# MarSaKi/VLN-BEVBert

Hardware: AMD Instinct MI355X
Metric: pretrain_samples_per_sec (higher is better)
Workload: dtype bf16+fp32-residual

## Files before the change

### include/bevbert_hip.h

```cpp
#ifndef BEVBERT_HIP_H
#define BEVBERT_HIP_H

#include <stdint.h>

#ifdef __cplusplus
extern "C" {
#endif

typedef struct ihipStream_t* hipStream_t;

#define BEVBERT_F32 0
#define BEVBERT_BF16 1
#define BEVBERT_F16 2

const char* bevbert_last_error(void);
int bevbert_version(void);
int bevbert_hip_error_reset(void);
const char* bevbert_arch(void);
const char* bevbert_attn_last_path(int backward);

int bevbert_bev_lift_bin(const float* depths, const float* T_c2w, const float* T_w2c, const float* S_w2c,
                         const float* pix_scale, int B, int V, int hw, float depth_scale, int dim, float res,
                         float y_clip, int* cell, int* order, int* cell_start, hipStream_t stream);
int bevbert_bev_bin_points(const float* points, const uint8_t* drop_mask, int B, int P, int dim, float res,
                           float y_clip, int* cell, int* order, int* cell_start, hipStream_t stream);
int bevbert_bev_splat_mean(const void* feat, int feat_dtype, const int* order, const int* cell_start, void* out,
                           int out_dtype, int B, int P, int K, int C, const uint8_t* sem_ids, const double* sem_dense,
                           int S, uint8_t* out_sem, uint8_t* out_sem_mask, const int* sample_rows, int rows_per_sample,
                           hipStream_t stream);

int bevbert_attn_fwd(const void* q, const void* k, const void* v, void* o, float* lse, const float* key_mask,
                     const float* bias, const int64_t* strides, int B, int nh, int Lq, int Lk, int head_dim,
                     float scale, int dtype, int impl, float drop_p, uint64_t seed, uint64_t offset,
                     uint64_t* drop_bits, int bits_ready, hipStream_t stream);
int bevbert_attn_bwd(const void* q, const void* k, const void* v, const void* o, const void* dout, const float* lse,
                     float* delta_ws, void* dq, void* dk, void* dv, float* dbias, const float* key_mask,
                     const float* bias, const int64_t* strides, int B, int nh, int Lq, int Lk, int head_dim,
                     float scale, int dtype, int impl, float drop_p, uint64_t seed, uint64_t offset,
                     const uint64_t* drop_bits, hipStream_t stream);
int64_t bevbert_attn_drop_bits_words(int B, int nh, int Lq, int Lk);
int bevbert_attn_drop_bits(uint64_t* drop_bits, int B, int nh, int Lq, int Lk, float drop_p, uint64_t seed,
                           uint64_t offset, hipStream_t stream);

int bevbert_bias_dropout_residual_layernorm_fwd(const void* x, const float* bias, const void* residual,
                                                const float* gamma, const float* beta, void* y, void* z_out,
                                                float* mean, float* rstd, int rows, int H, float eps, int dtype,
                                                float drop_p, uint64_t seed, uint64_t offset, hipStream_t stream);
int bevbert_layernorm_post_fwd(const void* x, const float* bias, const float* gamma, const float* beta,
                               const void* post1, const void* post2, void* y, void* z_out, float* mean, float* rstd,
                               int rows, int H, float eps, int dtype, hipStream_t stream);
int bevbert_layernorm_bwd(const void* dy, const void* z, const float* mean, const float* rstd, const float* gamma,
                          void* dz, void* dx, float* dgamma, float* dbeta, float* dbias, float* workspace, int rows,
                          int H, int dtype, float drop_p, uint64_t seed, uint64_t offset, int accumulate,
                          hipStream_t stream);
int bevbert_layernorm_bwd_add(const void* dy, const void* z, const float* mean, const float* rstd, const float* gamma,
                              void* dz, void* dx, const void* dz_add, float* dgamma, float* dbeta, float* dbias,
                              float* workspace, int rows, int H, int dtype, float drop_p, uint64_t seed, uint64_t offset,
                              int accumulate, hipStream_t stream);
int bevbert_layernorm_res32_fwd(const void* x, const float* bias, const void* residual, int residual_dtype,
                                const float* gamma, const float* beta, void* y16, float* y32, float* z32, float* mean,
                                float* rstd, int rows, int H, float eps, float drop_p, uint64_t seed, uint64_t offset,
                                hipStream_t stream);
// ... 180 lines not shown
```

### vln_bevbert_amd/csrc/attn_common.h

```cpp
#pragma once
#include "common.h"

#define ATTN_D 64

struct AttnArgs {
  const void *q, *k, *v;
  void* o;
  float* lse;
  const float* key_mask;
  const float* bias;
  int64_t ldq, ldk, ldv, ldo;
  int64_t bsq, bsk, bsv, bso;
  int B, nh, Lq, Lk;
  float scale;
  float drop_p;
  float keep_scale;
  uint32_t drop_thr;
  uint32_t drop_key;
  const uint32_t* salt;
  int nblk;
  int Lk2;
  uint64_t* drop_bits;
  uint64_t* drop_bits_b;
  int nq16, nk64;
  const void* dout;
  const float* delta;
  void *dq, *dk, *dv;
  float* dbias;
  int dbg;
};

__device__ __forceinline__ void attn_decode_block(const AttnArgs& a, int& blk, int& h, int& b) {
  const int nwg = gridDim.x, id = blockIdx.x;
  const int q = nwg >> 3, r = nwg & 7, xcd = id & 7, slot = id >> 3;
  const int w = (xcd < r ? xcd * (q + 1) : r * (q + 1) + (xcd - r) * q) + slot;
  blk = w % a.nblk;
  const int t = w / a.nblk;
  h = t % a.nh;
  b = t / a.nh;
}

__device__ __forceinline__ size_t attn_bits_word(const AttnArgs& a, int bh, int q16, int k64, int t, int r) {
  return ((((size_t)bh * a.nq16 + q16) * a.nk64 + k64) * 4 + t) * 4 + r;
}

__device__ __forceinline__ uint32_t attn_row_base(const AttnArgs& a, int b, int h, int q) {
  return (uint32_t)((((uint32_t)b * a.nh + h) * a.Lq + q) * (uint32_t)a.Lk2);
}
__device__ __forceinline__ uint32_t attn_elem(const AttnArgs& a, int b, int h, int q, int k) {
  return attn_row_base(a, b, h, q) + (uint32_t)k;
}
```

### vln_bevbert_amd/csrc/attn_short.hip

```cpp
#include "attn_mfma_common.h"

typedef const __attribute__((address_space(4))) uint64_t* sh_cu64p;

template <int CTRL> __device__ __forceinline__ float sh_dpp(float v) {
  return __int_as_float(__builtin_amdgcn_update_dpp(0, __float_as_int(v), CTRL, 0xf, 0xf, true));
}
__device__ __forceinline__ float sh_sum8(float v) {
  v += sh_dpp<0xB1>(v);
  v += sh_dpp<0x4E>(v);
  return v + sh_dpp<0x141>(v);
}
__device__ __forceinline__ bf16x8 sh_join(uint2 a, uint2 b) { return as_bf16x8(make_uint4(a.x, a.y, b.x, b.y)); }
__device__ __forceinline__ uint2 sh_pack4(const f32x4& v) {
  return make_uint2(pack_bf16x2(v[0], v[1]), pack_bf16x2(v[2], v[3]));
}
template <bool HI>
__device__ __forceinline__ bf16x8 sh_frag_tr(const bf16_raw* img, int stride, int row_lo, int row_hi, int col0, int lane) {
  const int i = lane & 15;
  const int off = (i >> 2) * stride + col0 + 4 * (i & 3);
  const uint2 lo = lds_tr16(img + row_lo * stride + off);
  uint2 hi = make_uint2(0u, 0u);
  if (HI) hi = lds_tr16(img + row_hi * stride + off);
  return as_bf16x8(make_uint4(lo.x, lo.y, hi.x, hi.y));
}

#define SH_ST_LD 72
__device__ __forceinline__ void sh_store_tile(bf16_raw* stage, const f32x4 (&acc)[4], float mul, bf16_raw* gtile, int64_t ld,
                                              int nrows, int lane) {
  const int g = lane >> 4, c = lane & 15;
#pragma unroll
  for (int dt = 0; dt < 4; ++dt)
    *reinterpret_cast<uint2*>(stage + c * SH_ST_LD + dt * 16 + g * 4) =
        make_uint2(pack_bf16x2(acc[dt][0] * mul, acc[dt][1] * mul), pack_bf16x2(acc[dt][2] * mul, acc[dt][3] * mul));
#pragma unroll
  for (int i = 0; i < 2; ++i) {
    const int row = (lane >> 3) + 8 * i, ch = lane & 7;
    const uint4 v = *reinterpret_cast<const uint4*>(stage + row * SH_ST_LD + ch * 8);
    if (row < nrows) *reinterpret_cast<uint4*>(gtile + (size_t)row * ld + ch * 8) = v;
  }
}

template <int NKT, int DROP>
__global__ __launch_bounds__(512) void attn_short_fwd_kernel(AttnArgs a) {
  constexpr int NC = (NKT + 1) / 2;
  __shared__ __attribute__((aligned(16))) bf16_raw s_k[16 * NKT * LDT];
  __shared__ __attribute__((aligned(16))) bf16_raw s_v[16 * NKT * LDT];
  __shared__ __attribute__((aligned(16))) float s_mk[16 * NKT];
  extern __shared__ __attribute__((aligned(16))) bf16_raw s_stage[];
  const int tid = threadIdx.x, lane = tid & 63, g = lane >> 4, c = lane & 15;
  const int w = __builtin_amdgcn_readfirstlane(tid >> 6), nw = blockDim.x >> 6;
  int blk, h, b;
  attn_decode_block(a, blk, h, b);
  const int bh = b * a.nh + h;
  if (DROP == 1) a.drop_key = bb_salted(a.drop_key, a.salt);
  const bf16_raw* qp = (const bf16_raw*)a.q + (size_t)b * a.bsq + h * ATTN_D;
  const bf16_raw* kp = (const bf16_raw*)a.k + (size_t)b * a.bsk + h * ATTN_D;
  const bf16_raw* vp = (const bf16_raw*)a.v + (size_t)b * a.bsv + h * ATTN_D;
  const float sc2 = a.scale * LOG2E, inv_sc2 = 1.0f / sc2;

  const int qt = blk * nw + w;
  const int qrow = qt * 16 + c;
  const int qr = qrow < a.Lq ? qrow : a.Lq - 1;
  bf16x8 qf[2];
// ... 182 lines not shown
      if (row < 16 * NQT) {
        *reinterpret_cast<uint4*>(s_q + row * LDT + ch * 8) = qv[i];
        *reinterpret_cast<uint4*>(s_do + row * LDT + ch * 8) = dv[i];
        const uint32_t dw[4] = {dv[i].x, dv[i].y, dv[i].z, dv[i].w}, ow[4] = {ov[i].x, ov[i].y, ov[i].z, ov[i].w};
        float dsum = 0.f;
#pragma unroll
        for (int j = 0; j < 4; ++j)
          dsum += __uint_as_float(dw[j] << 16) * __uint_as_float(ow[j] << 16) +
                  __uint_as_float(dw[j] & 0xffff0000u) * __uint_as_float(ow[j] & 0xffff0000u);
        dsum = sh_sum8(dsum);
        if ((lane & 7) == 0) s_dlt[row] = dsum;
      }
    }
  }
  if (tid < 16 * NQT) s_lse2[tid] = tid < a.Lq ? a.lse[(size_t)bh * a.Lq + tid] * LOG2E : INFINITY;
  if (tid < 16 * NKT) {
    float m = -INFINITY;
    if (tid < a.Lk) m = a.key_mask ? a.key_mask[(size_t)b * a.Lk + tid] * LOG2E : 0.f;
    s_mk[tid] = m;
  }
  __syncthreads();

  const f32x4 zero = (f32x4){0.f, 0.f, 0.f, 0.f};
  f32x4 dk[4], dv[4];
  if (w < NKT) {
    const bf16x8 kb0 = lds_frag_rows(s_k, t, 0, lane), kb1 = lds_frag_rows(s_k, t, 1, lane);
    const float mk2 = s_mk[t * 16 + c];
  #pragma unroll
    for (int dt = 0; dt < 4; ++dt) dk[dt] = dv[dt] = zero;
#pragma unroll
    for (int m = 0; m < NCQ; ++m) {
      uint2 pp[2] = {make_uint2(0u, 0u), make_uint2(0u, 0u)}, pds[2] = {make_uint2(0u, 0u), make_uint2(0u, 0u)};
#pragma unroll
      for (int j = 0; j < 2; ++j) {
        const int qt = 2 * m + j;
        if (qt < NQT) {
          f32x4 s = mfma16(lds_frag_rows(s_q, qt, 0, lane), kb0, zero);
          s = mfma16(lds_frag_rows(s_q, qt, 1, lane), kb1, s);
          f32x4 dp = mfma16(lds_frag_rows(s_do, qt, 0, lane), vb[0], zero);
          dp = mfma16(lds_frag_rows(s_do, qt, 1, lane), vb[1], dp);
          const float4 l4 = *reinterpret_cast<const float4*>(s_lse2 + 16 * qt + 4 * g);
          const float4 d4 = *reinterpret_cast<const float4*>(s_dlt + 16 * qt + 4 * g);
          const float lrow[4] = {l4.x, l4.y, l4.z, l4.w}, drow[4] = {d4.x, d4.y, d4.z, d4.w};
          uint32_t kbits = 0xfu;
          if (DROP) kbits = (uint32_t)(bw[qt < NQT ? qt : 0] >> (16 * (c >> 2) + 4 * g));
          f32x4 pd, dsv;
// ... 28 lines not shown
  }
  __syncthreads();
  constexpr bool STAGED = NR * 16 * SH_ST_LD * 2 <= 2 * 16 * NQT * LDT * 2;
  bf16_raw* const stage = s_q + w * 16 * SH_ST_LD;
  if (w < NKT) {
    const int key = t * 16 + c;
    if (STAGED) {
      if (t * 16 < a.Lk && !(a.dbg & 1)) {
        bf16_raw* dkp = (bf16_raw*)a.dk + (size_t)b * a.bsk + (size_t)(t * 16) * a.ldk + h * ATTN_D;
        bf16_raw* dvp = (bf16_raw*)a.dv + (size_t)b * a.bsv + (size_t)(t * 16) * a.ldv + h * ATTN_D;
        sh_store_tile(stage, dk, a.scale, dkp, a.ldk, a.Lk - t * 16, lane);
        sh_store_tile(stage, dv, 1.0f, dvp, a.ldv, a.Lk - t * 16, lane);
      }
    } else if (key < a.Lk && !((a.dbg & 1) && lane != 0)) {
      bf16_raw* dkp = (bf16_raw*)a.dk + (size_t)b * a.bsk + (size_t)key * a.ldk + h * ATTN_D;
      bf16_raw* dvp = (bf16_raw*)a.dv + (size_t)b * a.bsv + (size_t)key * a.ldv + h * ATTN_D;
#pragma unroll
      for (int dt = 0; dt < 4; ++dt) {
        st4<bf16_raw>(dkp + dt * 16 + g * 4, make_float4(dk[dt][0] * a.scale, dk[dt][1] * a.scale, dk[dt][2] * a.scale,
                                                          dk[dt][3] * a.scale));
        st4<bf16_raw>(dvp + dt * 16 + g * 4, make_float4(dv[dt][0], dv[dt][1], dv[dt][2], dv[dt][3]));
      }
    }
  }
  if (w < NQT && w * 16 < a.Lq) {
    const int qt = w;
    f32x4 dq[4];
#pragma unroll
    for (int dt = 0; dt < 4; ++dt) dq[dt] = zero;
#pragma unroll
    for (int m = 0; m < NCK; ++m) {
      if (2 * m + 1 < NKT) {
        const bf16x8 dsf = sh_frag_tr<true>(s_ds, DS_LD, 32 * m + 4 * g, 32 * m + 16 + 4 * g, 16 * qt, lane);
#pragma unroll
        for (int dt = 0; dt < 4; ++dt)
          dq[dt] = mfma16(sh_frag_tr<true>(s_k, LDT, 32 * m + 4 * g, 32 * m + 16 + 4 * g, dt * 16, lane), dsf, dq[dt]);
      } else {
        const bf16x8 dsf = sh_frag_tr<false>(s_ds, DS_LD, 32 * m + 4 * g, 0, 16 * qt, lane);
#pragma unroll
        for (int dt = 0; dt < 4; ++dt)
          dq[dt] = mfma16(sh_frag_tr<false>(s_k, LDT, 32 * m + 4 * g, 0, dt * 16, lane), dsf, dq[dt]);
      }
    }
    const int qrow = qt * 16 + c;
    if (STAGED) {
      if (!(a.dbg & 1)) {
        bf16_raw* dqp = (bf16_raw*)a.dq + (size_t)b * a.bsq + (size_t)(qt * 16) * a.ldq + h * ATTN_D;
        sh_store_tile(stage, dq, a.scale, dqp, a.ldq, a.Lq - qt * 16, lane);
      }
    } else if (qrow < a.Lq && !((a.dbg & 1) && lane != 0)) {
      bf16_raw* dqp = (bf16_raw*)a.dq + (size_t)b * a.bsq + (size_t)qrow * a.ldq + h * ATTN_D;
#pragma unroll
      for (int dt = 0; dt < 4; ++dt)
        st4<bf16_raw>(dqp + dt * 16 + g * 4, make_float4(dq[dt][0] * a.scale, dq[dt][1] * a.scale,
                                                          dq[dt][2] * a.scale, dq[dt][3] * a.scale));
    }
  }
}

#define SH_MAX_LEN 96

static bool sh_aligned(const AttnArgs& a) {
  return a.ldq % 8 == 0 && a.ldk % 8 == 0 && a.ldv % 8 == 0 && a.ldo % 8 == 0 && a.bsq % 8 == 0 && a.bsk % 8 == 0 &&
         a.bsv % 8 == 0 && a.bso % 8 == 0 && ((uintptr_t)a.q % 16) == 0 && ((uintptr_t)a.k % 16) == 0 &&
         ((uintptr_t)a.v % 16) == 0 && ((uintptr_t)a.o % 16) == 0;
}

static int sh_round_tiles(int n) {
  return n <= 2 ? 2 : n <= 3 ? 3 : n <= 5 ? 5 : 6;
}

static bool sh_on() {
  const char* v = getenv("BEVBERT_ATTN_SHORT");
  return !(v && v[0] == '0');
}

bool attn_short_fwd_supported(const AttnArgs& a, bool bits_ready) {
  if (!sh_on()) return false;
// ... 72 lines not shown
```

### vln_bevbert_amd/csrc/capi.hip

```cpp
#include <stdarg.h>

#include "attn_common.h"

static thread_local char g_err[512] = "";

void bb_set_error(const char* fmt, ...) {
  va_list ap;
  va_start(ap, fmt);
  vsnprintf(g_err, sizeof(g_err), fmt, ap);
  va_end(ap);
}

BEVBERT_API const char* bevbert_last_error(void) { return g_err; }
BEVBERT_API int bevbert_hip_error_reset(void) {
  int n = 0;
  while (hipGetLastError() != hipSuccess && n < 16) ++n;
  return n;
}

BEVBERT_API int bevbert_zero(void* p, int64_t bytes, hipStream_t stream) {
  BB_REQUIRE(p != nullptr && bytes >= 0, "zero: null pointer or negative size");
  if (bytes == 0) return BB_OK;
  hipError_t e = hipMemsetAsync(p, 0, (size_t)bytes, stream);
  if (e != hipSuccess) {
    bb_set_error("zero: hipMemsetAsync failed: %s", hipGetErrorString(e));
    return BB_ELAUNCH;
  }
  return BB_OK;
}

BEVBERT_API int bevbert_version(void) { return 112; }

static const uint32_t* g_step_salt = nullptr;
const uint32_t* bb_step_salt() { return g_step_salt; }
BEVBERT_API int bevbert_set_step_salt(const void* device_word) {
  g_step_salt = static_cast<const uint32_t*>(device_word);
  return BB_OK;
}
BEVBERT_API const char* bevbert_arch(void) { return "gfx950"; }

int attn_simple_fwd(const AttnArgs& a, int dtype, hipStream_t st);
int attn_simple_bwd(const AttnArgs& a, int dtype, hipStream_t st);
int attn_delta(const AttnArgs& a, float* delta, int dtype, hipStream_t st);
int attn_mfma_fwd(const AttnArgs& a, hipStream_t st);
int attn_mfma_bwd(const AttnArgs& a, hipStream_t st);
int attn_mfma_bwd1(const AttnArgs& a, hipStream_t st);
bool attn_mfma_bwd1_supported(const AttnArgs& a);
int attn_fwd2(const AttnArgs& a, hipStream_t st);
bool attn_fwd2_supported(const AttnArgs& a);
int attn_drop_bits(const AttnArgs& a, uint64_t* bits_f, uint64_t* bits_b, uint32_t* bits_l, hipStream_t st);
int attn_fwd4(const AttnArgs& a, const uint32_t* bits_l, hipStream_t st);
bool attn_fwd4_supported(const AttnArgs& a, const uint32_t* bits_l);
int attn_bwd2(const AttnArgs& a, hipStream_t st);
bool attn_bwd2_supported(const AttnArgs& a);
// ... 69 lines not shown
  const int im = pick_impl(dtype, impl);
  if (im == 2 || im == 3) {
    BB_REQUIRE(dtype == BB_BF16, "attn_fwd: the MFMA path takes bf16 tensors");
    static const bool gen1 = [] { const char* v = getenv("BEVBERT_ATTN_FWD"); return v && v[0] == '1'; }();
    if (!gen1 && !small_kernels_on() && attn_short_fwd_supported(a, bits_ready != 0))
      return ATTN_PATH(0, "attn_short_fwd", attn_short_fwd(a, bits_ready != 0, stream));
    if (!gen1 && small_kernels_on() && attn_small_fwd_supported(a)) return ATTN_PATH(0, "attn_small_fwd", attn_small_fwd(a, stream));
    const bool small = drop_p > 0.f && (int64_t)Lq * Lk < 32768 && Lk <= 256 && !bits_ready;
    if (!gen1 && !small && attn_fwd2_supported(a)) {
      uint32_t* bits_l = drop_bits ? reinterpret_cast<uint32_t*>(drop_bits + 2 * bits_words_one(B, nh, Lq, Lk)) : nullptr;
      if (drop_p > 0.f && !bits_ready) {
        rc = attn_drop_bits(a, a.drop_bits, a.drop_bits_b, bits_l, stream);
        if (rc != BB_OK) return rc;
      }
      if (attn_fwd4_supported(a, bits_l)) return ATTN_PATH(0, "attn_fwd4", attn_fwd4(a, bits_l, stream));
      return ATTN_PATH(0, "attn_fwd2", attn_fwd2(a, stream));
    }
    return ATTN_PATH(0, "attn_mfma_fwd", attn_mfma_fwd(a, stream));
  }
  if (attn_f32_supported(a, dtype, false)) return ATTN_PATH(0, "attn_f32_fwd", attn_f32_fwd(a, stream));
  return ATTN_PATH(0, "attn_simple_fwd", attn_simple_fwd(a, dtype, stream));
}

BEVBERT_API int bevbert_attn_bwd(const void* q, const void* k, const void* v, const void* o, const void* dout,
                                 const float* lse, float* delta_ws, void* dq, void* dk, void* dv, float* dbias,
                                 const float* key_mask, const float* bias, const int64_t* strides, int B, int nh,
                                 int Lq, int Lk, int head_dim, float scale, int dtype, int impl, float drop_p,
                                 uint64_t seed, uint64_t offset, const uint64_t* drop_bits, hipStream_t stream) {
  AttnArgs a;
  int rc = fill_common(a, q, k, v, key_mask, bias, strides, B, nh, Lq, Lk, head_dim, scale, drop_p, seed, offset);
  if (rc != BB_OK) return rc;
  a.drop_bits = const_cast<uint64_t*>(drop_bits);
  a.drop_bits_b = drop_bits ? a.drop_bits + bits_words_one(B, nh, Lq, Lk) : nullptr;
  BB_REQUIRE(dtype == BB_F32 || dtype == BB_BF16, "attn_bwd: dtype %d unsupported", dtype);
  BB_REQUIRE(lse != nullptr && delta_ws != nullptr, "attn_bwd: lse and the (B,nh,Lq) delta workspace are required");
  a.o = const_cast<void*>(o); a.dout = dout; a.lse = const_cast<float*>(lse); a.delta = delta_ws;
  a.dq = dq; a.dk = dk; a.dv = dv; a.dbias = dbias;
  const int im = pick_impl(dtype, impl);
  if (im == 2 || im == 3) {
    BB_REQUIRE(dtype == BB_BF16, "attn_bwd: the MFMA path takes bf16 tensors");
    static const bool split = [] { const char* v = getenv("BEVBERT_ATTN_BWD"); return v && v[0] == 's'; }();
    static const bool gen1 = [] { const char* v = getenv("BEVBERT_ATTN_BWD"); return v && v[0] == '1'; }();
    if (!split && !gen1 && im == 2 && !small_kernels_on() && attn_short_bwd_supported(a))
      return ATTN_PATH(1, "attn_short_bwd", attn_short_bwd(a, stream));
    if (!split && !gen1 && im == 2 && small_bwd2_on() && attn_small_bwd2_supported(a)) return ATTN_PATH(1, "attn_small_bwd2", attn_small_bwd2(a, stream));
    if (!split && !gen1 && small_kernels_on() && im == 2 && attn_small_bwd_supported(a)) return ATTN_PATH(1, "attn_small_bwd", attn_small_bwd(a, stream));
    static const bool gen3 = [] { const char* v = getenv("BEVBERT_ATTN_BWD3"); return !(v && v[0] == '0'); }();
    if (!split && !gen1 && gen3 && im == 2 && attn_bwd3_supported(a)) return ATTN_PATH(1, "attn_bwd3", attn_bwd3(a, stream));
    if (!split && !gen1 && im == 2 && attn_bwd2_supported(a)) return ATTN_PATH(1, "attn_bwd2", attn_bwd2(a, stream));
    if (!split && im == 2 && attn_mfma_bwd1_supported(a)) return ATTN_PATH(1, "attn_mfma_bwd1", attn_mfma_bwd1(a, stream));
    return ATTN_PATH(1, "attn_mfma_bwd", attn_mfma_bwd(a, stream));
  }
  rc = attn_delta(a, delta_ws, dtype, stream);
  if (rc != BB_OK) return rc;
  if (attn_f32_supported(a, dtype, true)) return ATTN_PATH(1, "attn_f32_bwd", attn_f32_bwd(a, stream));
  return ATTN_PATH(1, "attn_simple_bwd", attn_simple_bwd(a, dtype, stream));
}

__global__ void keep_mask_kernel(uint8_t* out, size_t n, uint32_t key, uint32_t thr, const uint32_t* salt) {
  key = bb_salted(key, salt);
  for (size_t i = (size_t)blockIdx.x * 256 + threadIdx.x; i < n; i += (size_t)gridDim.x * 256)
    out[i] = (uint8_t)bb_keep(key, (uint32_t)i, thr);
}
BEVBERT_API int64_t bevbert_attn_drop_bits_words(int B, int nh, int Lq, int Lk) {
  return 3 * bits_words_one(B, nh, Lq, Lk);
}

// ... 22 lines not shown
```

### vln_bevbert_amd/lib.py

```python
import ctypes
import os
import re
import subprocess

import torch

_HERE = os.path.dirname(os.path.abspath(__file__))
LIB_PATH = os.path.join(_HERE, "libbevbert_hip.so")
CSRC = os.path.join(_HERE, "csrc")
EXTRA_FLAGS = {"attn_fwd4.hip": ["-fno-slp-vectorize"]}
SOURCES = ["splat.hip", "rowops.hip", "attn_simple.hip", "attn_f32.hip", "attn_mfma.hip", "attn_bwd1.hip", "attn_fwd2.hip", "attn_fwd4.hip", "attn_bwd2.hip", "attn_bwd3.hip", "attn_small.hip", "attn_short.hip", "smallk.hip", "sap_loss.hip", "graph_nav.hip", "nav_expert.hip", "gemm.hip", "capi.hip"]
HEADER = os.path.join(os.path.dirname(_HERE), "include", "bevbert_hip.h")

F32, BF16, F16 = 0, 1, 2
_DT = {torch.float32: F32, torch.bfloat16: BF16, torch.float16: F16}


class BevBertHipError(RuntimeError):
    pass


def dtype_code(t):
    try:
        return _DT[t.dtype if torch.is_tensor(t) else t]
# ... 23 lines not shown
            print(" ".join(cmd), flush=True)
        subprocess.run(cmd, check=True, cwd=CSRC)

    with ThreadPoolExecutor(max_workers=min(8, max(1, len(jobs)))) as ex:
        list(ex.map(run, jobs))
    run([hipcc, "--offload-arch=gfx950", "-shared", "-fPIC", "-o", LIB_PATH] + objs + ["-lhipblaslt"])
    return LIB_PATH


def header_symbols():
    with open(HEADER) as f:
        return sorted(set(re.findall(r"\b(bevbert_\w+)\s*\(", f.read())))


_lib = None
_P, _I, _I64, _U64, _F = ctypes.c_void_p, ctypes.c_int, ctypes.c_int64, ctypes.c_uint64, ctypes.c_float

_PROTOS = {
    "bevbert_bev_lift_bin": [_P, _P, _P, _P, _P, _I, _I, _I, _F, _I, _F, _F, _P, _P, _P, _P],
    "bevbert_bev_bin_points": [_P, _P, _I, _I, _I, _F, _F, _P, _P, _P, _P],
    "bevbert_bev_splat_mean": [_P, _I, _P, _P, _P, _I, _I, _I, _I, _I, _P, _P, _I, _P, _P, _P, _I, _P],
    "bevbert_attn_fwd": [_P, _P, _P, _P, _P, _P, _P, _P, _I, _I, _I, _I, _I, _F, _I, _I, _F, _U64, _U64, _P, _I, _P],
    "bevbert_attn_drop_bits": [_P, _I, _I, _I, _I, _F, _U64, _U64, _P],
    "bevbert_attn_bwd": [_P, _P, _P, _P, _P, _P, _P, _P, _P, _P, _P, _P, _P, _P, _I, _I, _I, _I, _I, _F, _I, _I, _F,
                         _U64, _U64, _P, _P],
    "bevbert_bias_dropout_residual_layernorm_fwd": [_P, _P, _P, _P, _P, _P, _P, _P, _P, _I, _I, _F, _I, _F, _U64,
                                                    _U64, _P],
    "bevbert_layernorm_post_fwd": [_P, _P, _P, _P, _P, _P, _P, _P, _P, _P, _I, _I, _F, _I, _P],
    "bevbert_layernorm_bwd": [_P, _P, _P, _P, _P, _P, _P, _P, _P, _P, _P, _I, _I, _I, _F, _U64, _U64, _I, _P],
    "bevbert_layernorm_res32_fwd": [_P, _P, _P, _I, _P, _P, _P, _P, _P, _P, _P, _I, _I, _F, _F, _U64, _U64, _P],
    "bevbert_layernorm_res32_bwd": [_P, _P, _P, _P, _P, _P, _P, _P, _P, _P, _P, _P, _I, _I, _F, _U64, _U64, _I, _I, _P],
    "bevbert_colsum_any": [_P, _P, _I, _I, _I, _I, _P],
    "bevbert_sem_select": [_P, _P, _I, _I, _I, _P, _P, _P, _P],
    "bevbert_bce_rows_fwd": [_P, _P, _P, _P, _I, _I, _I, _P],
    "bevbert_bce_rows_bwd": [_P, _P, _P, _P, _P, _I, _I, _I, _P],
    "bevbert_weighted_mean_fwd": [_P, _P, _P, _F, _I, _P, _P],
    "bevbert_weighted_mean_bwd": [_P, _P, _P, _F, _I, _P, _P],
    "bevbert_layernorm_bwd_add": [_P, _P, _P, _P, _P, _P, _P, _P, _P, _P, _P, _P, _I, _I, _I, _F, _U64, _U64, _I, _P],
    "bevbert_embed_sum_layernorm_fwd": [_P, _P, _P, _P, _P, _P, _P, _P, _P, _P, _I, _I, _I, _F, _I, _F, _U64, _U64, _P],
    "bevbert_embedding_grad": [_P, _P, _P, _I, _I, _I, _I, _P],
    "bevbert_rows_gather": [_P, _P, _P, _I, _I, _I, _P],
    "bevbert_graph_bias_fwd": [_P, _P, _P, _P, _I64, _P],
    "bevbert_graph_bias_bwd": [_P, _P, _I, _I, _I, _I, _P, _P, _P, _P],
    "bevbert_smallk_linear_layernorm_fwd": [_P] * 11 + [_I, _I, _I, _F, _I, _P],
    "bevbert_smallk_linear_layernorm_bwd": [_P] * 12 + [_I, _I, _I, _I, _P],
    "bevbert_rows_scatter": [_P, _P, _P, _I, _I, _I, _I, _P],
# ... 122 lines not shown
```

### vln_bevbert_amd/ops_attention.py

```python
import math
import os as _os

import torch

from .lib import dtype_code, ptr, stream
from .ops_core import ATTN_BITS, HEAD_DIM, RT, _drop_bits_words, _mark_touched, _sink, call


def _strides(q, k, v, o):
    for t in (q, k, v, o):
        assert t.dim() == 3 and t.stride(2) == 1, "attention operands are (B, L, nh*64) with unit inner stride"
    import ctypes
    arr = (ctypes.c_int64 * 8)(q.stride(1), k.stride(1), v.stride(1), o.stride(1),
                               q.stride(0), k.stride(0), v.stride(0), o.stride(0))
    return arr


class _Attention(torch.autograd.Function):

    @staticmethod
    def forward(ctx, mode, a, b_, c_, key_mask, bias, nh, drop_p, impl):
        if mode == "self":
            H = a.shape[-1] // 3
            q, k, v = a[..., :H], a[..., H:2 * H], a[..., 2 * H:]
        elif mode == "cross":
            H = a.shape[-1]
            q, k, v = a, b_[..., :H], b_[..., H:]
        else:
            H = a.shape[-1]
# ... 37 lines not shown
            dq, dk, dv = da[..., :H], da[..., H:2 * H], da[..., 2 * H:]
            grads = (da, None, None)
        elif mode == "cross":
            H = a.shape[-1]
            q, k, v = a, b_[..., :H], b_[..., H:]
            dq = torch.empty_like(a)
            dkv = ctx.kv_slot[0].grad_slice(ctx.kv_slot[1], b_) if ctx.kv_slot is not None else torch.empty_like(b_)
            dk, dv = dkv[..., :H], dkv[..., H:]
            grads = (dq, dkv, None)
        else:
            q, k, v = a, b_, c_
            dq, dk, dv = torch.empty_like(a), torch.empty_like(b_), torch.empty_like(c_)
            grads = (dq, dk, dv)
        B, Lq, Lk = q.shape[0], q.shape[1], k.shape[1]
        delta = torch.empty(B, nh, Lq, dtype=torch.float32, device=q.device)
        slot = ctx.bias_slot
        if bias is not None and ctx.needs_input_grad[5] and slot is not None and Lq == Lk:
            dbias_h = slot[0].slot(slot[1], B, Lq, q.device)
        else:
            slot = None
            dbias_h = torch.zeros(B, nh, Lq, Lk, dtype=torch.float32, device=q.device) \
                if (bias is not None and ctx.needs_input_grad[5]) else None
        assert do.shape == o.shape
        call("bevbert_attn_bwd", ptr(q), ptr(k), ptr(v), ptr(o), ptr(do), ptr(lse), ptr(delta), ptr(dq), ptr(dk),
             ptr(dv), ptr(dbias_h), ptr(key_mask), ptr(bias), _strides(q, k, v, o), B, nh, Lq, Lk, HEAD_DIM, scale,
             dtype_code(q), impl, drop_p, seed, off, ptr(bits), stream())
        if slot is not None:
            dbias = slot[0].dummy
        else:
            dbias = None if dbias_h is None else dbias_h.sum(1)
        return (None,) + grads + (None, dbias, None, None, None)


class _BiasGradHolder:

    def __init__(self, layers, nh):
        self.layers, self.nh, self.buf, self.dummy = layers, nh, None, None

    def slot(self, i, B, G, device):
        if self.buf is None:
            self.buf = torch.empty(self.layers, B, self.nh, G, G, dtype=torch.float32, device=device)
            call("bevbert_zero", ptr(self.buf), self.buf.numel() * 4, stream())
            self.dummy = torch.zeros((), dtype=torch.float32, device=device).expand(B, G, G)
        return self.buf[i]


class _GraphBias(torch.autograd.Function):

    @staticmethod
    def forward(ctx, dists, weight, bias, layers, nh):
        dists = dists.to(torch.float32).contiguous()
        out = torch.empty_like(dists)
        call("bevbert_graph_bias_fwd", ptr(dists), ptr(weight), ptr(bias), ptr(out), dists.numel(), stream())
        ctx.save_for_backward(dists)
# ... 64 lines not shown
```

### vln_bevbert_amd/ops_gemm.py

```python
import os as _os

import torch
import torch.nn.functional as F

from . import lib
from .lib import dtype_code, ptr, stream
from .ops_core import RT, _LT_WS_BYTES, _compute, _gemm, _mark_touched, _sink, call
from .ops_reduce import ReduceQueue, WgradStream, _on_launch_stream, _partial_rows


_LT_ENABLED = _os.environ.get("BEVBERT_LT_GEMM", "1") == "1"


_LT_AUTOTUNE = int(_os.environ.get("BEVBERT_LT_AUTOTUNE", "32"))


_LT_UNSUPPORTED = set()


_LT_PLAN_BUDGET = int(_os.environ.get("BEVBERT_LT_PLAN_BUDGET", "8192"))


_LT_PLANS = {}


GEMM_FALLBACKS = {}


def _warn_fallback(kind, M, N, K, why="no direct hipBLASLt plan"):
    key = (kind, int(M), int(N), int(K))
    n = GEMM_FALLBACKS.get(key, 0)
# ... 156 lines not shown
    M, N = dy2.shape
    K = x2.shape[1]
    if dy2.dtype == torch.float32 and not (_LT_ENABLED and dy2.is_cuda):
        if dy2.is_cuda:
            _warn_fallback("wgrad", N, K, M, "BEVBERT_LT_GEMM=0")
        _gemm("wgrad", lambda: _on_launch_stream(lambda: sink.addmm_(dy2.t(), x2)), N, K, M)
        return None
    S = _split_k(M, N, K) if dy2.dtype != torch.float32 else 1
    if not (S > 1 and dy2.is_contiguous() and x2.is_contiguous()):
        S = 1
    batched = WgradStream.DEFER_FINALIZE and (N * K) % 4 == 0 and dy2.is_cuda
    part = _gemm("wgrad", lambda: _linear_wgrad(dy2, x2, S, scratch=batched), N, K, M)
    if batched:
        ReduceQueue.add_accum(part.data_ptr(), sink.data_ptr(), S, N * K, dtype_code(part))
        WgradStream._keep.append(part)
        return None
    if (N * K) % 4 == 0:
        call("bevbert_accum_partials", ptr(part), ptr(sink), S, N * K, dtype_code(part), stream())
    else:
        _on_launch_stream(lambda: sink.add_(part if S == 1 else part.sum(0)))
    return part


def _param_grads(w_sink, b_sink, dyc, xc):
    if w_sink is not None:
        part = _wgrad_into(w_sink, dyc, xc)
        if part is not None and lib._override is not None:
            WgradStream._keep.append(part)
    if b_sink is not None:
        C = dyc.shape[1]
        if WgradStream.DEFER_FINALIZE and dyc.shape[0] > 0:
            nb = _partial_rows(dyc.shape[0])
            part = RT.scratch.alloc(nb * C * 4, dyc.device)
            call("bevbert_colsum_partials", ptr(dyc), part, dyc.shape[0], C, dtype_code(dyc), stream())
            ReduceQueue.add(part, nb, 1, C, (ptr(b_sink), None, None))
        else:
            ws = RT.workspace(dyc.device, lib.load().bevbert_colsum_workspace_floats(C))
            call("bevbert_colsum", ptr(dyc), ptr(b_sink), ptr(ws), dyc.shape[0], C, dtype_code(dyc), 1, stream())


class _Linear(torch.autograd.Function):

    @staticmethod
    def forward(ctx, x, weight, bias, w_c, b_c, tap=False):
        y = _gemm("fwd", lambda: _linear_fwd(x, w_c, b_c), x.numel() // x.shape[-1], w_c.shape[0], w_c.shape[1])
        ctx.save_for_backward(x, w_c)
        ctx.params = (weight, bias)
        ctx.tap = tap
        ctx.set_materialize_grads(False)
        return (y, x.view_as(x)) if tap else y

    @staticmethod
# ... 16 lines not shown
            if C % 4 != 0:
                dyc = dy2 if dy2.is_contiguous() else dy2.contiguous()
                if b_sink is not None and dyc.is_cuda:
                    _mark_touched(bias)
                    call("bevbert_colsum_any", ptr(dyc), ptr(b_sink), dyc.shape[0], C, dtype_code(dyc), 1, stream())
                    b_sink = None
                elif b_sink is not None:
                    _mark_touched(bias)
                    b_sink.add_(dy2.float().sum(0))
                    b_sink = None
                else:
                    gb = dy2.float().sum(0).to(bias.dtype)
            else:
                ws = RT.workspace(dy.device, lib.load().bevbert_colsum_workspace_floats(C))
                dyc = dy2 if dy2.is_contiguous() else dy2.contiguous()
                t = torch.empty(C, dtype=torch.float32, device=dy.device)
                call("bevbert_colsum", ptr(dyc), ptr(t), ptr(ws), dyc.shape[0], C, dtype_code(dyc), 0, stream())
                gb = t.to(bias.dtype)
        if w_sink is not None or b_sink is not None:
            dyc = dy2 if dy2.is_contiguous() else dy2.contiguous()
            xc = x2 if x2.is_contiguous() else x2.contiguous()
            if w_sink is not None:
                _mark_touched(weight)
            if b_sink is not None:
                _mark_touched(bias)
            WgradStream.submit(dy.device, lambda: _param_grads(w_sink, b_sink, dyc, xc), dyc, xc, dy)
        return dx, gw, gb, None, None, None


def linear(x, weight, bias=None, w_c=None, b_c=None):
    if w_c is None:
        w_c = _compute(weight)
    if bias is not None and b_c is None:
        b_c = _compute(bias)
    return _Linear.apply(x, weight, bias, w_c, b_c)


def linear_res(x, weight, bias=None):
    if not (x.requires_grad and torch.is_grad_enabled()) or getattr(x, "_res32", None) is not None:
        return linear(x, weight, bias), x
    return _Linear.apply(x, weight, bias, _compute(weight), None if bias is None else _compute(bias), True)


class _PackedParam:

    def __init__(self, params, compute, main_grad):
        self.params, self.compute, self.main_grad = params, compute, main_grad
        self.requires_grad = any(p.requires_grad for p in params)
        self.dtype = params[0].dtype
# ... 10 lines not shown
        ctx.save_for_backward(x)
        ctx.packed = (pw, pb)
        y = _gemm("fwd", lambda: _linear_fwd(x, pw.compute, pb.compute), x.numel() // x.shape[-1],
                  pw.compute.shape[0], pw.compute.shape[1])
        ctx.set_materialize_grads(False)
        return (y, x.view_as(x)) if tap else y

    @staticmethod
    def backward(ctx, dy, dres=None):
        (x,) = ctx.saved_tensors
        pw, pb = ctx.packed
        if dy is None:
            return dres, None, None, None
        dy2 = dy.reshape(-1, dy.shape[-1])
        x2 = x.reshape(-1, x.shape[-1])
        M, N, K = dy2.shape[0], dy2.shape[1], x2.shape[1]
        dx = _gemm("dgrad", lambda: _linear_dgrad(dy2, pw.compute, dres), M, K, N).view(x.shape) if ctx.needs_input_grad[0] else None
        if pw.requires_grad:
            pw.touch()
            pb.touch()
            C = dy2.shape[1]
            dyc = dy2 if dy2.is_contiguous() else dy2.contiguous()
            xc = x2 if x2.is_contiguous() else x2.contiguous()
            WgradStream.submit(dy.device, lambda: _param_grads(pw.main_grad, pb.main_grad, dyc, xc), dyc, xc, dy)
        return dx, None, None, None


def linear_packed(x, pw, pb):
    return _LinearPacked.apply(x, pw, pb)


HOIST_KV = _os.environ.get("BEVBERT_HOIST_KV", "1") == "1"


class _KVGradHolder:

    def __init__(self, n_layers, width):
        self.n, self.width, self.buf = n_layers, width, None

    def grad_slice(self, layer, like):
        if self.buf is None:
            self.buf = torch.empty(like.shape[:-1] + (self.n * self.width,), dtype=like.dtype, device=like.device)
        return self.buf[..., layer * self.width:(layer + 1) * self.width]


class _HoistedKV(torch.autograd.Function):

    @staticmethod
    def forward(ctx, x, pw, pb, n_layers):
        ctx.save_for_backward(x)
        ctx.packed = (pw, pb)
        y = _gemm("fwd", lambda: _linear_fwd(x, pw.compute, pb.compute), x.numel() // x.shape[-1],
                  pw.compute.shape[0], pw.compute.shape[1])
        width = y.shape[-1] // n_layers
        ctx.holder = _KVGradHolder(n_layers, width)
        return tuple(y[..., i * width:(i + 1) * width] for i in range(n_layers))

    @staticmethod
    def backward(ctx, *grads):
        (x,) = ctx.saved_tensors
        pw, pb = ctx.packed
        h = ctx.holder
        some = next((g for g in grads if g is not None), None)
        if some is None:
            return None, None, None, None
        for i, g in enumerate(grads):
            dst = h.grad_slice(i, some)
            if g is None:
                dst.zero_()
            elif g.data_ptr() != dst.data_ptr() or g.stride() != dst.stride():
                dst.copy_(g)
        dy2 = h.buf.reshape(-1, h.buf.shape[-1])
        x2 = x.reshape(-1, x.shape[-1])
        M, N, K = dy2.shape[0], dy2.shape[1], x2.shape[1]
        dx = _gemm("dgrad", lambda: _linear_dgrad(dy2, pw.compute), M, K, N).view(x.shape) if ctx.needs_input_grad[0] else None
        if pw.requires_grad:
            pw.touch()
            pb.touch()
            xc = x2 if x2.is_contiguous() else x2.contiguous()
            WgradStream.submit(dy2.device, lambda: _param_grads(pw.main_grad, pb.main_grad, dy2, xc), dy2, xc, h.buf)
        return dx, None, None, None


def hoisted_kv(context, pw, pb, n_layers):
    outs = _HoistedKV.apply(context, pw, pb, n_layers)
    if torch.is_grad_enabled() and any(o.requires_grad for o in outs):
        holder = outs[0].grad_fn.holder if hasattr(outs[0].grad_fn, "holder") else None
        if holder is not None:
            for i, o in enumerate(outs):
                o._kv_grad_slot = (holder, i)
    return outs


def linear_packed_res(x, pw, pb):
    if not (x.requires_grad and torch.is_grad_enabled()) or getattr(x, "_res32", None) is not None:
        return _LinearPacked.apply(x, pw, pb), x
    return _LinearPacked.apply(x, pw, pb, True)


def gemm_plan_count():
    return int(lib.load().bevbert_gemm_plan_count())
```

### vln_bevbert_amd/ops_reduce.py

```python
import math
import os as _os

import torch

from . import lib
from .lib import stream
from .ops_core import ATTN_BITS, Branches, RT, call


def join_captured_side_streams(extra=()):
    if not torch.cuda.is_available() or not torch.cuda.is_current_stream_capturing():
        return 0
    cur = torch.cuda.current_stream()
    seen, n = {cur.cuda_stream}, 0
    cands = [ATTN_BITS.stream] + list(Branches._streams.values()) + list(WgradStream.streams) + list(extra)
    for st in cands:
        if st is None or st.cuda_stream in seen:
            continue
        seen.add(st.cuda_stream)
        with torch.cuda.stream(st):
            capturing = torch.cuda.is_current_stream_capturing()
        if capturing:
            cur.wait_stream(st)
            n += 1
# ... 80 lines not shown
    def flush_all(cls):
        if ReduceQueue.jobs or ReduceQueue.accum_jobs:
            dev = torch.device("cuda", torch.cuda.current_device())
            if cls.active(dev):
                h = lib.stream()
                slot = cls._pending.get(h)
                if slot is None:
                    slot = cls._pending[h] = (torch.cuda.current_stream(dev), [])
                slot[1].append(lambda: ReduceQueue.flush(dev))
                mine = slot
                for other in cls._pending.values():
                    if other is not mine:
                        cls._flush(other)
                cls._flush(mine, final=True)
                return
            ReduceQueue.wait_producers(torch.cuda.current_stream(dev))
            ReduceQueue.flush(dev)
        for slot in cls._pending.values():
            cls._flush(slot)

    @classmethod
    def release(cls):
        cls._keep.clear()

    @classmethod
    def drop_pending(cls):
        for _, fns in cls._pending.values():
            fns.clear()
        cls._keep.clear()


class ScratchRing:

    INITIAL = 256 << 20

    def __init__(self, nbytes=1 << 30, max_total=64 << 30):
        self.nbytes = nbytes
        self.max_total = max(max_total, nbytes)
        self.size = 0
        self.buf = None
        self.base = 0
        self.off = 0
        self.ci = 0
        self._chunks = []
        self._old = []

    def reset(self):
        self.off = self.ci = 0
        if self._chunks:
            self.buf, self.base, self.size = self._chunks[0]

    def total_bytes(self):
# ... 214 lines not shown
```

Baseline: 3628.

## Fuse bias-gradient column sums of dQ/dK/dV into short attention backward kernel

The short attention backward kernel now also computes per-batch column sums of dQ, dK and dV, rounded to bf16, through DPP reductions and an LDS pass. These are written as partial rows into scratch buffers. The Python side arms these buffers before the call and registers them under the gradient tensor's identity. Downstream linear backward paths then feed the precomputed partials to the bias reduction instead of re-reading the full dy. This removes a separate pass over the gradient activations for the QKV bias grads, at the cost of extra kernel work, a barrier, thread-local C state and key matching on data pointers.

```diff
diff --git a/include/bevbert_hip.h b/include/bevbert_hip.h
--- a/include/bevbert_hip.h
+++ b/include/bevbert_hip.h
@@ -38,6 +38,8 @@
                      const float* bias, const int64_t* strides, int B, int nh, int Lq, int Lk, int head_dim,
                      float scale, int dtype, int impl, float drop_p, uint64_t seed, uint64_t offset,
                      const uint64_t* drop_bits, hipStream_t stream);
+int bevbert_attn_bwd_bias_partials(float* part_q, float* part_k, float* part_v, int64_t ldq, int64_t ldkv, int rows_cap);
+int bevbert_attn_bias_partial_rows(int* rows);
 int64_t bevbert_attn_drop_bits_words(int B, int nh, int Lq, int Lk);
 int bevbert_attn_drop_bits(uint64_t* drop_bits, int B, int nh, int Lq, int Lk, float drop_p, uint64_t seed,
                            uint64_t offset, hipStream_t stream);
diff --git a/vln_bevbert_amd/csrc/attn_common.h b/vln_bevbert_amd/csrc/attn_common.h
--- a/vln_bevbert_amd/csrc/attn_common.h
+++ b/vln_bevbert_amd/csrc/attn_common.h
@@ -28,6 +28,8 @@
   void *dq, *dk, *dv;
   float* dbias;
   int dbg;
+  float *cs_q, *cs_k, *cs_v;
+  int64_t cs_ldq, cs_ldkv;
 };
 
 __device__ __forceinline__ void attn_decode_block(const AttnArgs& a, int& blk, int& h, int& b) {
diff --git a/vln_bevbert_amd/csrc/attn_short.hip b/vln_bevbert_amd/csrc/attn_short.hip
--- a/vln_bevbert_amd/csrc/attn_short.hip
+++ b/vln_bevbert_amd/csrc/attn_short.hip
@@ -39,6 +39,25 @@
     if (row < nrows) *reinterpret_cast<uint4*>(gtile + (size_t)row * ld + ch * 8) = v;
   }
 }
+
+__device__ __forceinline__ float sh_tile_colsum(const f32x4 (&acc)[4], float mul, int nrows, int lane) {
+  const int c = lane & 15;
+  const bool live = c < nrows;
+  float out = 0.f;
+#pragma unroll
+  for (int dt = 0; dt < 4; ++dt)
+#pragma unroll
+    for (int r = 0; r < 4; ++r) {
+      float v = live ? __uint_as_float(pack_bf16x2(acc[dt][r] * mul, 0.f) << 16) : 0.f;
+      v += sh_dpp<0xB1>(v);
+      v += sh_dpp<0x4E>(v);
+      v += sh_dpp<0x141>(v);
+      v += sh_dpp<0x140>(v);
+      out = c == dt * 4 + r ? v : out;
+    }
+  return out;
+}
+__device__ __forceinline__ int sh_colsum_col(int lane) { return 16 * ((lane & 15) >> 2) + 4 * (lane >> 4) + (lane & 3); }
 
 template <int NKT, int DROP>
 __global__ __launch_bounds__(512) void attn_short_fwd_kernel(AttnArgs a) {
@@ -267,6 +286,8 @@
   __syncthreads();
 
   const f32x4 zero = (f32x4){0.f, 0.f, 0.f, 0.f};
+  const bool sums = a.cs_q != nullptr || a.cs_k != nullptr;
+  float cs_q = 0.f, cs_k = 0.f, cs_v = 0.f;
   f32x4 dk[4], dv[4];
   if (w < NKT) {
     const bf16x8 kb0 = lds_frag_rows(s_k, t, 0, lane), kb1 = lds_frag_rows(s_k, t, 1, lane);
@@ -341,6 +362,10 @@
         st4<bf16_raw>(dvp + dt * 16 + g * 4, make_float4(dv[dt][0], dv[dt][1], dv[dt][2], dv[dt][3]));
       }
     }
+    if (sums && t * 16 < a.Lk) {
+      cs_k = sh_tile_colsum(dk, a.scale, a.Lk - t * 16, lane);
+      cs_v = sh_tile_colsum(dv, 1.0f, a.Lk - t * 16, lane);
+    }
   }
   if (w < NQT && w * 16 < a.Lq) {
     const int qt = w;
@@ -373,6 +398,30 @@
       for (int dt = 0; dt < 4; ++dt)
         st4<bf16_raw>(dqp + dt * 16 + g * 4, make_float4(dq[dt][0] * a.scale, dq[dt][1] * a.scale,
                                                           dq[dt][2] * a.scale, dq[dt][3] * a.scale));
+    }
+    if (sums) cs_q = sh_tile_colsum(dq, a.scale, a.Lq - qt * 16, lane);
+  }
+  if (sums) {
+    float* const s_cs = reinterpret_cast<float*>(sm);
+    static_assert(3 * NR * 64 * 4 <= L::bytes, "column-sum image exceeds the kernel's LDS");
+    asm volatile("s_waitcnt lgkmcnt(0)" : : : "memory");
+    __builtin_amdgcn_s_barrier();
+    const int col = sh_colsum_col(lane);
+    if (w < NQT) s_cs[w * 64 + col] = cs_q;
+    if (w < NKT) {
+      s_cs[(NR + w) * 64 + col] = cs_k;
+      s_cs[(2 * NR + w) * 64 + col] = cs_v;
+    }
+    asm volatile("s_waitcnt lgkmcnt(0)" : : : "memory");
+    __builtin_amdgcn_s_barrier();
+    for (int i = tid; i < 3 * 64; i += 64 * NR) {
+      const int which = i >> 6, d = i & 63;
+      float* const dst = which == 0 ? a.cs_q : which == 1 ? a.cs_k : a.cs_v;
+      if (dst == nullptr) continue;
+      const int nt = ((which == 0 ? a.Lq : a.Lk) + 15) >> 4;
+      float s = 0.f;
+      for (int j = 0; j < nt; ++j) s += s_cs[(which * NR + j) * 64 + d];
+      dst[(size_t)b * (which == 0 ? a.cs_ldq : a.cs_ldkv) + h * ATTN_D + d] = s;
     }
   }
 }
diff --git a/vln_bevbert_amd/csrc/capi.hip b/vln_bevbert_amd/csrc/capi.hip
--- a/vln_bevbert_amd/csrc/capi.hip
+++ b/vln_bevbert_amd/csrc/capi.hip
@@ -29,7 +29,7 @@
   return BB_OK;
 }
 
-BEVBERT_API int bevbert_version(void) { return 112; }
+BEVBERT_API int bevbert_version(void) { return 113; }
 
 static const uint32_t* g_step_salt = nullptr;
 const uint32_t* bb_step_salt() { return g_step_salt; }
@@ -145,11 +145,35 @@
   return ATTN_PATH(0, "attn_simple_fwd", attn_simple_fwd(a, dtype, stream));
 }
 
+struct AttnColsums {
+  float *q, *k, *v;
+  int64_t ldq, ldkv;
+  int rows_cap;
+};
+static thread_local AttnColsums g_cs = {nullptr, nullptr, nullptr, 0, 0, 0};
+static thread_local int g_cs_rows = 0;
+
+BEVBERT_API int bevbert_attn_bwd_bias_partials(float* part_q, float* part_k, float* part_v, int64_t ldq, int64_t ldkv,
+                                               int rows_cap) {
+  BB_REQUIRE(ldq % 4 == 0 && ldkv % 4 == 0 && ldq >= 0 && ldkv >= 0, "attn_bwd_bias_partials: row strides %lld / %lld",
+             (long long)ldq, (long long)ldkv);
+  g_cs = {part_q, part_k, part_v, ldq, ldkv, rows_cap};
+  return BB_OK;
+}
+BEVBERT_API int bevbert_attn_bias_partial_rows(int* rows) {
+  BB_REQUIRE(rows != nullptr, "attn_bias_partial_rows: null output");
+  *rows = g_cs_rows;
+  return BB_OK;
+}
+
 BEVBERT_API int bevbert_attn_bwd(const void* q, const void* k, const void* v, const void* o, const void* dout,
                                  const float* lse, float* delta_ws, void* dq, void* dk, void* dv, float* dbias,
                                  const float* key_mask, const float* bias, const int64_t* strides, int B, int nh,
                                  int Lq, int Lk, int head_dim, float scale, int dtype, int impl, float drop_p,
                                  uint64_t seed, uint64_t offset, const uint64_t* drop_bits, hipStream_t stream) {
+  const AttnColsums cs = g_cs;
+  g_cs = {nullptr, nullptr, nullptr, 0, 0, 0};
+  g_cs_rows = 0;
   AttnArgs a;
   int rc = fill_common(a, q, k, v, key_mask, bias, strides, B, nh, Lq, Lk, head_dim, scale, drop_p, seed, offset);
   if (rc != BB_OK) return rc;
@@ -164,8 +188,13 @@
     BB_REQUIRE(dtype == BB_BF16, "attn_bwd: the MFMA path takes bf16 tensors");
     static const bool split = [] { const char* v = getenv("BEVBERT_ATTN_BWD"); return v && v[0] == 's'; }();
     static const bool gen1 = [] { const char* v = getenv("BEVBERT_ATTN_BWD"); return v && v[0] == '1'; }();
-    if (!split && !gen1 && im == 2 && !small_kernels_on() && attn_short_bwd_supported(a))
-      return ATTN_PATH(1, "attn_short_bwd", attn_short_bwd(a, stream));
+    if (!split && !gen1 && im == 2 && !small_kernels_on() && attn_short_bwd_supported(a)) {
+      const bool sums = (cs.q || cs.k) && cs.rows_cap >= 1;
+      if (sums) { a.cs_q = cs.q; a.cs_k = cs.k; a.cs_v = cs.v; a.cs_ldq = cs.ldq; a.cs_ldkv = cs.ldkv; }
+      rc = attn_short_bwd(a, stream);
+      if (rc == BB_OK && sums) g_cs_rows = 1;
+      return ATTN_PATH(1, "attn_short_bwd", rc);
+    }
     if (!split && !gen1 && im == 2 && small_bwd2_on() && attn_small_bwd2_supported(a)) return ATTN_PATH(1, "attn_small_bwd2", attn_small_bwd2(a, stream));
     if (!split && !gen1 && small_kernels_on() && im == 2 && attn_small_bwd_supported(a)) return ATTN_PATH(1, "attn_small_bwd", attn_small_bwd(a, stream));
     static const bool gen3 = [] { const char* v = getenv("BEVBERT_ATTN_BWD3"); return !(v && v[0] == '0'); }();
diff --git a/vln_bevbert_amd/lib.py b/vln_bevbert_amd/lib.py
--- a/vln_bevbert_amd/lib.py
+++ b/vln_bevbert_amd/lib.py
@@ -69,6 +69,8 @@
     "bevbert_bev_splat_mean": [_P, _I, _P, _P, _P, _I, _I, _I, _I, _I, _P, _P, _I, _P, _P, _P, _I, _P],
     "bevbert_attn_fwd": [_P, _P, _P, _P, _P, _P, _P, _P, _I, _I, _I, _I, _I, _F, _I, _I, _F, _U64, _U64, _P, _I, _P],
     "bevbert_attn_drop_bits": [_P, _I, _I, _I, _I, _F, _U64, _U64, _P],
+    "bevbert_attn_bwd_bias_partials": [_P, _P, _P, _I64, _I64, _I],
+    "bevbert_attn_bias_partial_rows": [_P],
     "bevbert_attn_bwd": [_P, _P, _P, _P, _P, _P, _P, _P, _P, _P, _P, _P, _P, _P, _I, _I, _I, _I, _I, _F, _I, _I, _F,
                          _U64, _U64, _P, _P],
     "bevbert_bias_dropout_residual_layernorm_fwd": [_P, _P, _P, _P, _P, _P, _P, _P, _P, _I, _I, _F, _I, _F, _U64,
diff --git a/vln_bevbert_amd/ops_attention.py b/vln_bevbert_amd/ops_attention.py
--- a/vln_bevbert_amd/ops_attention.py
+++ b/vln_bevbert_amd/ops_attention.py
@@ -1,10 +1,13 @@
+import ctypes
 import math
 import os as _os
 
 import torch
 
+from . import lib
 from .lib import dtype_code, ptr, stream
 from .ops_core import ATTN_BITS, HEAD_DIM, RT, _drop_bits_words, _mark_touched, _sink, call
+from .ops_reduce import BiasPartials, ReduceQueue, WgradStream
 
 
 def _strides(q, k, v, o):
@@ -88,14 +91,61 @@
             dbias_h = torch.zeros(B, nh, Lq, Lk, dtype=torch.float32, device=q.device) \
                 if (bias is not None and ctx.needs_input_grad[5]) else None
         assert do.shape == o.shape
+        cs = _arm_bias_sums(mode, q, nh, B, Lq, Lk, bias, drop_p, impl)
         call("bevbert_attn_bwd", ptr(q), ptr(k), ptr(v), ptr(o), ptr(do), ptr(lse), ptr(delta), ptr(dq), ptr(dk),
              ptr(dv), ptr(dbias_h), ptr(key_mask), ptr(bias), _strides(q, k, v, o), B, nh, Lq, Lk, HEAD_DIM, scale,
              dtype_code(q), impl, drop_p, seed, off, ptr(bits), stream())
+        if cs is not None:
+            _publish_bias_sums(cs, mode, grads)
         if slot is not None:
             dbias = slot[0].dummy
         else:
             dbias = None if dbias_h is None else dbias_h.sum(1)
         return (None,) + grads + (None, dbias, None, None, None)
+
+
+_BIAS_ROWS = {}
+FUSED_BIAS_SUMS = _os.environ.get("BEVBERT_ATTN_BIAS_SUMS", "1") == "1"
+
+
+def attn_bias_partial_rows():
+    r = ctypes.c_int(0)
+    lib.call("bevbert_attn_bias_partial_rows", ctypes.addressof(r))
+    return r.value
+
+
+def _arm_bias_sums(mode, q, nh, B, Lq, Lk, bias, drop_p, impl):
+    if (mode == "sep" or q.dtype != torch.bfloat16 or not q.is_cuda or not WgradStream.DEFER_FINALIZE
+            or not FUSED_BIAS_SUMS):
+        return None
+    key = (mode, B, nh, Lq, Lk, bias is not None, drop_p > 0, impl)
+    rows = _BIAS_ROWS.get(key, 1)
+    if rows == 0:
+        return None
+    H = nh * HEAD_DIM
+    if mode == "self":
+        part = RT.scratch.alloc(B * rows * 3 * H * 4, q.device)
+        pq, pk, pv, ldq, ldkv = part, part + 4 * H, part + 8 * H, 3 * H, 3 * H
+    else:
+        pq = RT.scratch.alloc(B * rows * H * 4, q.device)
+        pk = RT.scratch.alloc(B * rows * 2 * H * 4, q.device)
+        pv, ldq, ldkv = pk + 4 * H, H, 2 * H
+    call("bevbert_attn_bwd_bias_partials", pq, pk, pv, ldq, ldkv, rows)
+    return key, B, pq, pk
+
+
+def _publish_bias_sums(cs, mode, grads):
+    key, B, pq, pk = cs
+    rows = attn_bias_partial_rows()
+    _BIAS_ROWS[key] = rows
+    if rows == 0:
+        return
+    ReduceQueue._note_producer()
+    if mode == "self":
+        BiasPartials.put(grads[0], pq, B * rows)
+    else:
+        BiasPartials.put(grads[0], pq, B * rows)
+        BiasPartials.put(grads[1], pk, B * rows)
 
 
 class _BiasGradHolder:
diff --git a/vln_bevbert_amd/ops_gemm.py b/vln_bevbert_amd/ops_gemm.py
--- a/vln_bevbert_amd/ops_gemm.py
+++ b/vln_bevbert_amd/ops_gemm.py
@@ -6,7 +6,7 @@
 from . import lib
 from .lib import dtype_code, ptr, stream
 from .ops_core import RT, _LT_WS_BYTES, _compute, _gemm, _mark_touched, _sink, call
-from .ops_reduce import ReduceQueue, WgradStream, _on_launch_stream, _partial_rows
+from .ops_reduce import BiasPartials, ReduceQueue, WgradStream, _on_launch_stream, _partial_rows
 
 
 _LT_ENABLED = _os.environ.get("BEVBERT_LT_GEMM", "1") == "1"
@@ -209,12 +209,15 @@
     return part
 
 
-def _param_grads(w_sink, b_sink, dyc, xc):
+def _param_grads(w_sink, b_sink, dyc, xc, b_parts=None):
     if w_sink is not None:
         part = _wgrad_into(w_sink, dyc, xc)
         if part is not None and lib._override is not None:
             WgradStream._keep.append(part)
-    if b_sink is not None:
+    if b_parts is not None:
+        for part, nb, C, out in b_parts:
+            ReduceQueue.add(part, nb, 1, C, (out, None, None))
+    elif b_sink is not None:
         C = dyc.shape[1]
         if WgradStream.DEFER_FINALIZE and dyc.shape[0] > 0:
             nb = _partial_rows(dyc.shape[0])
@@ -277,9 +280,13 @@
             xc = x2 if x2.is_contiguous() else x2.contiguous()
             if w_sink is not None:
                 _mark_touched(weight)
+            b_parts = None
             if b_sink is not None:
                 _mark_touched(bias)
-            WgradStream.submit(dy.device, lambda: _param_grads(w_sink, b_sink, dyc, xc), dyc, xc, dy)
+                pre = BiasPartials.take(dy)
+                if pre is not None:
+                    b_parts = [(pre[0], pre[1], C, b_sink.data_ptr())]
+            WgradStream.submit(dy.device, lambda: _param_grads(w_sink, b_sink, dyc, xc, b_parts), dyc, xc, dy)
         return dx, gw, gb, None, None, None
 
 
@@ -336,7 +343,9 @@
             C = dy2.shape[1]
             dyc = dy2 if dy2.is_contiguous() else dy2.contiguous()
             xc = x2 if x2.is_contiguous() else x2.contiguous()
-            WgradStream.submit(dy.device, lambda: _param_grads(pw.main_grad, pb.main_grad, dyc, xc), dyc, xc, dy)
+            pre = BiasPartials.take(dy)
+            b_parts = None if pre is None else [(pre[0], pre[1], C, pb.main_grad.data_ptr())]
+            WgradStream.submit(dy.device, lambda: _param_grads(pw.main_grad, pb.main_grad, dyc, xc, b_parts), dyc, xc, dy)
         return dx, None, None, None
 
 
@@ -378,12 +387,14 @@
         some = next((g for g in grads if g is not None), None)
         if some is None:
             return None, None, None, None
+        parts = []
         for i, g in enumerate(grads):
             dst = h.grad_slice(i, some)
             if g is None:
                 dst.zero_()
             elif g.data_ptr() != dst.data_ptr() or g.stride() != dst.stride():
                 dst.copy_(g)
+            parts.append(BiasPartials.take(dst) if g is not None else None)
         dy2 = h.buf.reshape(-1, h.buf.shape[-1])
         x2 = x.reshape(-1, x.shape[-1])
         M, N, K = dy2.shape[0], dy2.shape[1], x2.shape[1]
@@ -392,7 +403,12 @@
             pw.touch()
             pb.touch()
             xc = x2 if x2.is_contiguous() else x2.contiguous()
-            WgradStream.submit(dy2.device, lambda: _param_grads(pw.main_grad, pb.main_grad, dy2, xc), dy2, xc, h.buf)
+            b_parts = None
+            if all(p is not None for p in parts):
+                base = pb.main_grad.data_ptr()
+                b_parts = [(p[0], p[1], h.width, base + 4 * i * h.width) for i, p in enumerate(parts)]
+            WgradStream.submit(dy2.device, lambda: _param_grads(pw.main_grad, pb.main_grad, dy2, xc, b_parts), dy2, xc,
+                               h.buf)
         return dx, None, None, None
 
 
diff --git a/vln_bevbert_amd/ops_reduce.py b/vln_bevbert_amd/ops_reduce.py
--- a/vln_bevbert_amd/ops_reduce.py
+++ b/vln_bevbert_amd/ops_reduce.py
@@ -126,12 +126,36 @@
     @classmethod
     def release(cls):
         cls._keep.clear()
+        BiasPartials.clear()
 
     @classmethod
     def drop_pending(cls):
         for _, fns in cls._pending.values():
             fns.clear()
         cls._keep.clear()
+        BiasPartials.clear()
+
+
+class BiasPartials:
+
+    _by_key = {}
+
+    @staticmethod
+    def _key(t):
+        return t.data_ptr(), tuple(t.shape), tuple(t.stride())
+
+    @classmethod
+    def put(cls, grad, partials_ptr, nblocks):
+        cls._by_key[cls._key(grad)] = (grad, partials_ptr, nblocks)
+
+    @classmethod
+    def take(cls, grad):
+        e = cls._by_key.pop(cls._key(grad), None) if cls._by_key else None
+        return None if e is None else e[1:]
+
+    @classmethod
+    def clear(cls):
+        cls._by_key.clear()
 
 
 class ScratchRing:
```

Result: no change. 3616 (median of 2 runs) (-0.3%).
